# hippylib/hippyflow

Hardware: AMD Instinct MI355X
Metric: randomized-SVD throughput (GDoF*rank/s) (higher is better)
Workload: dtype f64

## Files before the change

### hippyflow_amd/csrc/hfmi_skinny.hip

```cpp
#include "hfmi_internal.h"

typedef double d4 __attribute__((ext_vector_type(4)));
typedef double d2 __attribute__((ext_vector_type(2)));
#define MFMA_F64(a, b, c) __builtin_amdgcn_mfma_f64_16x16x4f64((a), (b), (c), 0, 0, 0)
typedef const __attribute__((address_space(1))) d2* gd2ptr;
typedef const __attribute__((address_space(1))) double* gdptr;

#ifndef SS_NT
#define SS_NT 1
#endif
#if SS_NT
#define SS_LOAD(p) __builtin_nontemporal_load(p)
#else
#define SS_LOAD(p) (*(p))
#endif
#ifndef SS_PROBE
#define SS_PROBE 0
#endif
constexpr int SS_THREADS = 512;

template <int NT, int TPW, int NQ, bool STORE>
__device__ __forceinline__ void ss_stage(const double* __restrict__ L, double* __restrict__ Lnext, const int la,
                                         const int la1, const int (&toa)[TPW], const int (&tob)[TPW],
                                         d4 (&acc)[TPW], const d2 (&r)[NQ], const int dst0) {
  constexpr int CT = NQ * 32;
  constexpr int S = 4 * NT;
  constexpr int W0 = (S >= 8) ? (3 * S) / 4 : 0;
  constexpr int PER = (NQ + (S - W0) - 1) / (S - W0);
  d2 fa[2], fb[2];
  fa[0] = *reinterpret_cast<const d2*>(L + toa[0] + la);
  fb[0] = *reinterpret_cast<const d2*>(L + tob[0] + la);
#pragma unroll
  for (int st = 0; st < S; ++st) {
    if (st + 1 < S) {
      const int it = (st + 1) / NT, ti = (st + 1) % NT;
      const int lx = (it & 1) ? la1 : la;
      fa[(st + 1) & 1] = *reinterpret_cast<const d2*>(L + toa[ti] + lx + it * (8 * CT));
      fb[(st + 1) & 1] = *reinterpret_cast<const d2*>(L + tob[ti] + lx + it * (8 * CT));
    }
    if (STORE && st >= W0) {
#pragma unroll
      for (int j = 0; j < PER; ++j) {
        const int q = (st - W0) * PER + j;
        if (q < NQ) *reinterpret_cast<d2*>(Lnext + dst0 + q * 64) = r[q];
      }
    }
    __builtin_amdgcn_sched_barrier(0);
    const int ti = st % NT;
    acc[ti] = MFMA_F64(fa[st & 1].x, fb[st & 1].x, acc[ti]);
    acc[ti] = MFMA_F64(fa[st & 1].y, fb[st & 1].y, acc[ti]);
    __builtin_amdgcn_sched_barrier(0);
  }
}

__device__ __forceinline__ gdptr ss_colptr(int v, int ctot, int acols, const double* A, int64_t lda, int m,
                                           const double* B, int64_t ldb, int k) {
  const int vv = v < ctot ? v : ctot - 1;
  const double* p;
  if (vv < acols) {
    const int cc = vv < m ? vv : m - 1;
    p = A + (int64_t)cc * lda;
  } else {
    const int cc = (vv - acols) < k ? (vv - acols) : k - 1;
    p = B + (int64_t)cc * ldb;
  }
  return (gdptr)p;
}

template <int NT, int TPW, int NQ, int PF>
__device__ __forceinline__ void ss_main(double* __restrict__ lds, const gdptr* __restrict__ ptab,
                                        const gdptr (&ptr)[NQ], const int nstages, const int col0, const int off,
                                        const int dst0, const int la, const int la1, const int (&toa)[TPW],
                                        const int (&tob)[TPW], d4 (&acc)[TPW]) {
  constexpr int BUF = NQ * 32 * SS_BK;
  d2 reg[PF][NQ];
  auto stage_load = [&](d2(&r)[NQ], int s) {
    if (s > nstages - 1) s = nstages - 1;
#pragma unroll
    for (int q = 0; q < NQ; ++q) {
      if constexpr (PF == 2)
        r[q] = SS_LOAD(reinterpret_cast<gd2ptr>(ptr[q] + (int64_t)s * SS_BK));
      else
        r[q] = SS_LOAD(reinterpret_cast<gd2ptr>(ptab[col0 + 32 * q] + ((int64_t)s * SS_BK + off)));
    }
  };
  if (nstages > 0) {
    stage_load(reg[0], 0);
#pragma unroll
    for (int q = 0; q < NQ; ++q) *reinterpret_cast<d2*>(lds + dst0 + q * 64) = reg[0][q];
    if constexpr (PF == 2) stage_load(reg[0], 1);
    __syncthreads();
  }
  if constexpr (PF == 1) {
    for (int s = 0; s < nstages; ++s) {
      stage_load(reg[0], s + 1);
      __builtin_amdgcn_sched_barrier(0);
      ss_stage<NT, TPW, NQ, true>(lds + (s & 1) * BUF, lds + ((s + 1) & 1) * BUF, la, la1, toa, tob, acc, reg[0], dst0);
      __syncthreads();
    }
  } else {
    auto stage_store = [&](const d2(&r)[NQ]) {
#pragma unroll
      for (int q = 0; q < NQ; ++q) *reinterpret_cast<d2*>(lds + dst0 + q * 64) = r[q];
    };
    for (int s = 0; s < nstages; s += 2) {
      stage_load(reg[1], s + 2);
      __builtin_amdgcn_sched_barrier(0);
      ss_stage<NT, TPW, NQ, false>(lds, lds, la, la1, toa, tob, acc, reg[0], dst0);
      __syncthreads();
      stage_store(reg[0]);
      __syncthreads();
      if (s + 1 < nstages) {
        stage_load(reg[0], s + 3);
        __builtin_amdgcn_sched_barrier(0);
        ss_stage<NT, TPW, NQ, false>(lds, lds, la, la1, toa, tob, acc, reg[1], dst0);
        __syncthreads();
        stage_store(reg[1]);
        __syncthreads();
      }
    }
  }
}

template <int TPW, int NQ, int PF>
__global__ __launch_bounds__(SS_THREADS, (TPW <= 4 ? 4 : 2)) void k_tsgemm_ss(
    const double* __restrict__ A, int64_t lda, int m, int rt, const double* __restrict__ B, int64_t ldb, int k, int ct,
    int same, int64_t Npad, int64_t chunk, double* __restrict__ part) {
  extern __shared__ __attribute__((aligned(16))) char smem[];
  constexpr int CT = NQ * 32;
  constexpr int BUF = CT * SS_BK;
  double* lds = reinterpret_cast<double*>(smem);
  gdptr* ptab = reinterpret_cast<gdptr*>(lds + 2 * BUF);
  const int tid = threadIdx.x, lane = tid & 63;
  const int wave = __builtin_amdgcn_readfirstlane(tid >> 6);
  const int r16 = lane & 15, kk = lane >> 4;
  const int acols = rt * 16;
  const int ctot = same ? acols : acols + ct * 16;
  const int bcol0 = same ? 0 : acols;

  const int64_t t_begin = (int64_t)blockIdx.x * chunk;
  int64_t t_end = t_begin + chunk;
  if (t_end > Npad) t_end = Npad;
  const int nstages = t_end > t_begin ? (int)((t_end - t_begin) / SS_BK) : 0;

  const int col0 = tid >> 4;
  const int cq = tid & 15;
  const int dst0 = (cq * CT + (col0 ^ (cq & 7))) * 2;
  gdptr ptr[NQ];
#pragma unroll
  for (int q = 0; q < NQ; ++q) ptr[q] = nullptr;
  if constexpr (PF == 2) {
#pragma unroll
    for (int q = 0; q < NQ; ++q) ptr[q] = ss_colptr(col0 + 32 * q, ctot, acols, A, lda, m, B, ldb, k) + (t_begin + cq * 2);
  } else {
    for (int v = tid; v < CT; v += SS_THREADS) ptab[v] = ss_colptr(v, ctot, acols, A, lda, m, B, ldb, k) + t_begin;
    __syncthreads();
  }

  const int ntiles = same ? rt * (rt + 1) / 2 : rt * ct;
  const bool last_valid = wave + 8 * (TPW - 1) < ntiles;
  auto tile_rc = [&](int id, int& r, int& c) {
    if (same) {
      r = 0;
      while (id >= rt - r) {
        id -= rt - r;
        ++r;
      }
      c = r + id;
    } else {
      r = id / ct;
      c = id - r * ct;
    }
  };
  int toa[TPW], tob[TPW];
#pragma unroll
  for (int ti = 0; ti < TPW; ++ti) {
    int id = wave + 8 * ti;
    if (id > ntiles - 1) id = ntiles - 1;
    int r, c;
    tile_rc(id, r, c);
    toa[ti] = r * 32;
    tob[ti] = (bcol0 + c * 16) * 2;
  }
  const int la = (kk * CT + (r16 ^ kk)) * 2, la1 = (kk * CT + (r16 ^ (kk + 4))) * 2;
  d4 acc[TPW];
#pragma unroll
  for (int ti = 0; ti < TPW; ++ti) acc[ti] = d4{0.0, 0.0, 0.0, 0.0};

  if (TPW == 1 || last_valid)
    ss_main<TPW, TPW, NQ, PF>(lds, ptab, ptr, nstages, col0, cq * 2, dst0, la, la1, toa, tob, acc);
  else
    ss_main<(TPW > 1 ? TPW - 1 : 1), TPW, NQ, PF>(lds, ptab, ptr, nstages, col0, cq * 2, dst0, la, la1, toa, tob, acc);

  const int kpad = ct * 16;
  double* P = part + (int64_t)blockIdx.x * acols * kpad;
#pragma unroll
  for (int ti = 0; ti < TPW; ++ti) {
    const int id = wave + 8 * ti;
    if (id < ntiles) {
      int r, c;
      tile_rc(id, r, c);
#pragma unroll
      for (int e = 0; e < 4; ++e) P[(int64_t)(r * 16 + kk + 4 * e) * kpad + c * 16 + r16] = acc[ti][e];
      if (same && r != c) {
#pragma unroll
        for (int e = 0; e < 4; ++e) P[(int64_t)(c * 16 + r16) * kpad + r * 16 + kk + 4 * e] = acc[ti][e];
      }
    }
  }
}

template <int RB, int CB, int EN, int NQ>
__device__ __forceinline__ void ssb_stage(const double* __restrict__ L, double* __restrict__ Lnext, const int la, const int la1,
                                          const int (&toa)[RB], const int (&tob)[CB], const int (&etoa)[EN > 0 ? EN : 1],
                                          const int (&etob)[EN > 0 ? EN : 1], d4 (&acc)[RB][CB], d4 (&eacc)[EN > 0 ? EN : 1],
                                          const d2 (&r)[NQ], const int dst0, const int probe_acols = 0) {
  constexpr int CT = NQ * 32;
  constexpr int EA = EN > 0 ? EN : 1;
  (void)probe_acols;
  d2 fa[2][RB], fb[2][CB], ea[2][EA], eb[2][EA];
#pragma unroll
  for (int i = 0; i < RB; ++i) fa[0][i] = *reinterpret_cast<const d2*>(L + toa[i] + la);
#pragma unroll
  for (int j = 0; j < CB; ++j) fb[0][j] = *reinterpret_cast<const d2*>(L + tob[j] + la);
#pragma unroll
  for (int e = 0; e < EN; ++e) {
    ea[0][e] = *reinterpret_cast<const d2*>(L + etoa[e] + la);
    eb[0][e] = *reinterpret_cast<const d2*>(L + etob[e] + la);
  }
#pragma unroll
  for (int it = 0; it < 4; ++it) {
    if (it + 1 < 4) {
      const int lx = (((it + 1) & 1) ? la1 : la) + (it + 1) * (8 * CT);
#pragma unroll
      for (int i = 0; i < RB; ++i) fa[(it + 1) & 1][i] = *reinterpret_cast<const d2*>(L + toa[i] + lx);
#pragma unroll
      for (int j = 0; j < CB; ++j) {
#if SS_PROBE & 2
        fb[(it + 1) & 1][j] = d2{fb[it & 1][j].y, fb[it & 1][j].x};
#else
        fb[(it + 1) & 1][j] = *reinterpret_cast<const d2*>(L + tob[j] + lx);
#endif
      }
#pragma unroll
      for (int e = 0; e < EN; ++e) {
        ea[(it + 1) & 1][e] = *reinterpret_cast<const d2*>(L + etoa[e] + lx);
        eb[(it + 1) & 1][e] = *reinterpret_cast<const d2*>(L + etob[e] + lx);
      }
    }
    if (it >= 2) {
      constexpr int H = (NQ + 1) / 2;
#pragma unroll
      for (int q = (it - 2) * H; q < ((it - 2) * H + H < NQ ? (it - 2) * H + H : NQ); ++q) {
#if SS_PROBE & 1
        if ((int)(threadIdx.x >> 4) + 32 * q >= probe_acols) {
          asm volatile("" ::"v"(r[q].x), "v"(r[q].y));
          continue;
        }
#endif
        *reinterpret_cast<d2*>(Lnext + dst0 + q * 64) = r[q];
      }
    }
    __builtin_amdgcn_sched_barrier(0);
#pragma unroll
    for (int i = 0; i < RB; ++i)
#pragma unroll
      for (int j = 0; j < CB; ++j) acc[i][j] = MFMA_F64(fa[it & 1][i].x, fb[it & 1][j].x, acc[i][j]);
#pragma unroll
    for (int e = 0; e < EN; ++e) eacc[e] = MFMA_F64(ea[it & 1][e].x, eb[it & 1][e].x, eacc[e]);
#pragma unroll
    for (int i = 0; i < RB; ++i)
#pragma unroll
      for (int j = 0; j < CB; ++j) acc[i][j] = MFMA_F64(fa[it & 1][i].y, fb[it & 1][j].y, acc[i][j]);
#pragma unroll
    for (int e = 0; e < EN; ++e) eacc[e] = MFMA_F64(ea[it & 1][e].y, eb[it & 1][e].y, eacc[e]);
    __builtin_amdgcn_sched_barrier(0);
  }
}

template <int RB, int CB, int EN, int NQ>
__device__ __forceinline__ void ssb_stage_pipe(const double* __restrict__ L, double* __restrict__ Lnext, const int la, const int la1,
                                               const int (&toa)[RB], const int (&tob)[CB], const int (&etoa)[EN > 0 ? EN : 1],
                                               const int (&etob)[EN > 0 ? EN : 1], d4 (&acc)[RB][CB], d4 (&eacc)[EN > 0 ? EN : 1],
                                               const d2 (&r)[NQ], const int dst0, d2 (&fa)[2][RB], d2 (&fb)[2][CB],
                                               d2 (&ea)[2][EN > 0 ? EN : 1], d2 (&eb)[2][EN > 0 ? EN : 1], const int probe_acols = 0) {
  constexpr int CT = NQ * 32;
  (void)probe_acols;
#pragma unroll
  for (int it = 0; it < 4; ++it) {
    if (it == 3) __syncthreads();
    {
      const double* src = (it + 1 < 4) ? L : Lnext;
      const int g = (it + 1) & 3;
      const int lx = ((g & 1) ? la1 : la) + g * (8 * CT);
#pragma unroll
      for (int i = 0; i < RB; ++i) fa[(it + 1) & 1][i] = *reinterpret_cast<const d2*>(src + toa[i] + lx);
#pragma unroll
      for (int j = 0; j < CB; ++j) {
#if SS_PROBE & 2
        fb[(it + 1) & 1][j] = d2{fb[it & 1][j].y, fb[it & 1][j].x};
#else
        fb[(it + 1) & 1][j] = *reinterpret_cast<const d2*>(src + tob[j] + lx);
#endif
      }
#pragma unroll
      for (int e = 0; e < EN; ++e) {
        ea[(it + 1) & 1][e] = *reinterpret_cast<const d2*>(src + etoa[e] + lx);
        eb[(it + 1) & 1][e] = *reinterpret_cast<const d2*>(src + etob[e] + lx);
      }
    }
    if (it < 2) {
      constexpr int H = (NQ + 1) / 2;
#pragma unroll
      for (int q = it * H; q < (it * H + H < NQ ? it * H + H : NQ); ++q) {
#if SS_PROBE & 1
        if ((int)(threadIdx.x >> 4) + 32 * q >= probe_acols) {
          asm volatile("" ::"v"(r[q].x), "v"(r[q].y));
          continue;
        }
#endif
        *reinterpret_cast<d2*>(Lnext + dst0 + q * 64) = r[q];
      }
    }
    __builtin_amdgcn_sched_barrier(0);
#pragma unroll
    for (int i = 0; i < RB; ++i)
#pragma unroll
      for (int j = 0; j < CB; ++j) acc[i][j] = MFMA_F64(fa[it & 1][i].x, fb[it & 1][j].x, acc[i][j]);
#pragma unroll
    for (int e = 0; e < EN; ++e) eacc[e] = MFMA_F64(ea[it & 1][e].x, eb[it & 1][e].x, eacc[e]);
#pragma unroll
    for (int i = 0; i < RB; ++i)
#pragma unroll
      for (int j = 0; j < CB; ++j) acc[i][j] = MFMA_F64(fa[it & 1][i].y, fb[it & 1][j].y, acc[i][j]);
#pragma unroll
    for (int e = 0; e < EN; ++e) eacc[e] = MFMA_F64(ea[it & 1][e].y, eb[it & 1][e].y, eacc[e]);
    __builtin_amdgcn_sched_barrier(0);
  }
}

template <int RB, int CB, int EN, int NQ, int PF, int RT, bool PIPE>
__device__ __forceinline__ void ssb_run(double* __restrict__ lds, const gdptr* __restrict__ ptab, const int nstages, const int col0,
                                        const int off, const int dst0, const int la, const int la1, const int row_tile0,
                                        const int col_tile0, const int bcol0, double* __restrict__ P, const int kpad, const int r16,
                                        const int kk, const int ext0, const int ext_col0) {
  constexpr int BUF = NQ * 32 * SS_BK;
  constexpr int EA = EN > 0 ? EN : 1;
  int toa[RB], tob[CB], etoa[EA], etob[EA], er[EA], ec[EA];
#pragma unroll
  for (int i = 0; i < RB; ++i) toa[i] = (row_tile0 + i) * 32;
#pragma unroll
  for (int j = 0; j < CB; ++j) tob[j] = (bcol0 + (col_tile0 + j) * 16) * 2;
#pragma unroll
  for (int e = 0; e < EA; ++e) {
    const int id = ext0 + 8 * e;
    er[e] = id % RT;
    ec[e] = ext_col0 + id / RT;
    etoa[e] = er[e] * 32;
    etob[e] = (bcol0 + ec[e] * 16) * 2;
  }
  d4 acc[RB][CB], eacc[EA];
#pragma unroll
  for (int i = 0; i < RB; ++i)
#pragma unroll
    for (int j = 0; j < CB; ++j) acc[i][j] = d4{0.0, 0.0, 0.0, 0.0};
#pragma unroll
  for (int e = 0; e < EA; ++e) eacc[e] = d4{0.0, 0.0, 0.0, 0.0};
  d2 reg[PF][NQ];
  auto stage_load = [&](d2(&rr)[NQ], int s) {
    if (s > nstages - 1) s = nstages - 1;
#pragma unroll
    for (int q = 0; q < NQ; ++q) rr[q] = SS_LOAD(reinterpret_cast<gd2ptr>(ptab[col0 + 32 * q] + ((int64_t)s * SS_BK + off)));
  };
  if (nstages > 0) {
    stage_load(reg[0], 0);
#pragma unroll
    for (int q = 0; q < NQ; ++q) *reinterpret_cast<d2*>(lds + dst0 + q * 64) = reg[0][q];
    if constexpr (PF == 2) stage_load(reg[0], 1);
    __syncthreads();
  }
  if constexpr (PIPE) {
    d2 fa[2][RB], fb[2][CB], ea[2][EA], eb[2][EA];
#pragma unroll
    for (int i = 0; i < RB; ++i) fa[0][i] = *reinterpret_cast<const d2*>(lds + toa[i] + la);
#pragma unroll
    for (int j = 0; j < CB; ++j) fb[0][j] = *reinterpret_cast<const d2*>(lds + tob[j] + la);
#pragma unroll
    for (int e = 0; e < EN; ++e) {
      ea[0][e] = *reinterpret_cast<const d2*>(lds + etoa[e] + la);
      eb[0][e] = *reinterpret_cast<const d2*>(lds + etob[e] + la);
    }
    if constexpr (PF == 2) {
      for (int s = 0; s < nstages; s += 2) {
        stage_load(reg[1], s + 2);
        __builtin_amdgcn_sched_barrier(0);
        ssb_stage_pipe<RB, CB, EN, NQ>(lds, lds + BUF, la, la1, toa, tob, etoa, etob, acc, eacc, reg[0], dst0, fa, fb, ea, eb, RT * 16);
        if (s + 1 < nstages) {
          stage_load(reg[0], s + 3);
          __builtin_amdgcn_sched_barrier(0);
          ssb_stage_pipe<RB, CB, EN, NQ>(lds + BUF, lds, la, la1, toa, tob, etoa, etob, acc, eacc, reg[1], dst0, fa, fb, ea, eb, RT * 16);
        }
      }
    } else {
      for (int s = 0; s < nstages; ++s) {
        stage_load(reg[0], s + 1);
        __builtin_amdgcn_sched_barrier(0);
        ssb_stage_pipe<RB, CB, EN, NQ>(lds + (s & 1) * BUF, lds + ((s + 1) & 1) * BUF, la, la1, toa, tob, etoa, etob, acc, eacc,
                                       reg[0], dst0, fa, fb, ea, eb, RT * 16);
      }
    }
  } else if constexpr (PF == 2) {
    for (int s = 0; s < nstages; s += 2) {
      stage_load(reg[1], s + 2);
      __builtin_amdgcn_sched_barrier(0);
      ssb_stage<RB, CB, EN, NQ>(lds, lds + BUF, la, la1, toa, tob, etoa, etob, acc, eacc, reg[0], dst0, RT * 16);
      __syncthreads();
      if (s + 1 < nstages) {
        stage_load(reg[0], s + 3);
        __builtin_amdgcn_sched_barrier(0);
        ssb_stage<RB, CB, EN, NQ>(lds + BUF, lds, la, la1, toa, tob, etoa, etob, acc, eacc, reg[1], dst0, RT * 16);
        __syncthreads();
      }
    }
  } else {
    for (int s = 0; s < nstages; ++s) {
      stage_load(reg[0], s + 1);
      __builtin_amdgcn_sched_barrier(0);
      ssb_stage<RB, CB, EN, NQ>(lds + (s & 1) * BUF, lds + ((s + 1) & 1) * BUF, la, la1, toa, tob, etoa, etob, acc, eacc, reg[0], dst0, RT * 16);
      __syncthreads();
    }
  }
#pragma unroll
  for (int i = 0; i < RB; ++i)
#pragma unroll
    for (int j = 0; j < CB; ++j)
#pragma unroll
      for (int e = 0; e < 4; ++e)
        P[(int64_t)((row_tile0 + i) * 16 + kk + 4 * e) * kpad + (col_tile0 + j) * 16 + r16] = acc[i][j][e];
#pragma unroll
  for (int x = 0; x < EN; ++x)
#pragma unroll
    for (int e = 0; e < 4; ++e) P[(int64_t)(er[x] * 16 + kk + 4 * e) * kpad + ec[x] * 16 + r16] = eacc[x][e];
}

template <int RT, int CTL, int NQ, bool PIPE>
__global__ __launch_bounds__(SS_THREADS, 2) void k_tsgemm_ssb(const double* __restrict__ A, int64_t lda, int m,
                                                              const double* __restrict__ B, int64_t ldb, int k, int64_t Npad,
                                                              int64_t chunk, double* __restrict__ part) {
  extern __shared__ __attribute__((aligned(16))) char smem[];
  constexpr int CT = NQ * 32;
  constexpr int BUF = CT * SS_BK;
  constexpr int RB0 = (RT + 1) / 2, RB1 = RT / 2;
  constexpr int CBF = CTL / 4, CM = 4 * CBF, NLEFT = (CTL - CM) * RT;
  static_assert(RB1 >= 1 && CBF >= 1, "blocked variant needs at least 2 x 4 tiles");
  constexpr int ENB_HI = (NLEFT + 7) / 8, ENB_LO = NLEFT / 8 + ((NLEFT % 8) > 3 ? 1 : 0);
  constexpr int ENT_HI = (NLEFT + 3) / 8, ENT_LO = NLEFT > 4 ? (NLEFT - 4) / 8 + (((NLEFT - 4) % 8) > 3 ? 1 : 0) : 0;
  double* lds = reinterpret_cast<double*>(smem);
  gdptr* ptab = reinterpret_cast<gdptr*>(lds + 2 * BUF);
  const int tid = threadIdx.x, lane = tid & 63;
  const int wave = __builtin_amdgcn_readfirstlane(tid >> 6);
  const int r16 = lane & 15, kk = lane >> 4;
  constexpr int acols = RT * 16, ctot = (RT + CTL) * 16;
  const int64_t t_begin = (int64_t)blockIdx.x * chunk;
  int64_t t_end = t_begin + chunk;
  if (t_end > Npad) t_end = Npad;
  const int nstages = t_end > t_begin ? (int)((t_end - t_begin) / SS_BK) : 0;
  const int col0 = tid >> 4, cq = tid & 15;
  const int dst0 = (cq * CT + (col0 ^ (cq & 7))) * 2;
  for (int v = tid; v < CT; v += SS_THREADS) ptab[v] = ss_colptr(v, ctot, acols, A, lda, m, B, ldb, k) + t_begin;
  __syncthreads();
  const int la = (kk * CT + (r16 ^ kk)) * 2, la1 = (kk * CT + (r16 ^ (kk + 4))) * 2;
  const int rg = wave >> 2, cg = wave & 3;
  const int row_tile0 = rg ? RB0 : 0;
  const int col_tile0 = cg * CBF;
  const int ext0 = rg ? cg : cg + 4;
  int en = 0;
  for (int id = ext0; id < NLEFT; id += 8) ++en;
  constexpr int kpad = CTL * 16;
  double* P = part + (int64_t)blockIdx.x * acols * kpad;
  constexpr int PF = (RT * CTL <= 56) ? 2 : 1;
#define SSB_RUN(RBV, ENV) ssb_run<RBV, CBF, ENV, NQ, PF, RT, PIPE>(lds, ptab, nstages, col0, cq * 2, dst0, la, la1, row_tile0, col_tile0, acols, P, kpad, r16, kk, ext0, CM)
  if (rg == 0) {
    if (ENT_HI != ENT_LO && en == ENT_LO) SSB_RUN(RB0, ENT_LO);
    else SSB_RUN(RB0, ENT_HI);
  } else {
    if (ENB_HI != ENB_LO && en == ENB_LO) SSB_RUN(RB1, ENB_LO);
    else SSB_RUN(RB1, ENB_HI);
  }
#undef SSB_RUN
}

typedef void (*ss_kernel_t)(const double*, int64_t, int, int, const double*, int64_t, int, int, int, int64_t, int64_t, double*);
typedef void (*ssb_kernel_t)(const double*, int64_t, int, const double*, int64_t, int, int64_t, int64_t, double*);
static ss_kernel_t ss_kernel(const ss_plan& p) {
#define SS_CASE(T, Q) \
  if (p.tpw == T && p.nq == Q) return k_tsgemm_ss<T, Q, ss_pf(T, Q)>;
  HFMI_SS_CASES(SS_CASE)
#undef SS_CASE
  return nullptr;
}
static ssb_kernel_t ssb_kernel(const ss_plan& p) {
#define SSB_CASE(R, Cc) \
  if (p.rt == R && p.ct == Cc) return p.pipe ? k_tsgemm_ssb<R, Cc, (R + Cc + 1) / 2, true> : k_tsgemm_ssb<R, Cc, (R + Cc + 1) / 2, false>;
  HFMI_SSB_CASES(SSB_CASE)
#undef SSB_CASE
  return nullptr;
}

int launch_tsgemm_ss(hfmi_ctx* ctx, const double* A, int64_t lda, int m, const double* B, int64_t ldb, int k,
                     int64_t N, double scale, double beta, double* C, int64_t rs, int64_t cs, int nsplit_req) {
  const bool same = (A == B && lda == ldb && m == k);
  const ss_plan p = ss_plan_make(m, k, N, same, nsplit_req, tsgemm_knobs_ref(), ctx->num_cus);
  if (lda % 32 != 0 || ldb % 32 != 0 || lda < p.Npad || ldb < p.Npad)
    HFMI_FAIL(HFMI_ERR_INVALID, "tsgemm_ss: leading dimensions must be multiples of 32 and >= round_up(N,32)");
  const ss_kernel_t kern = p.blocked ? nullptr : ss_kernel(p);
  const ssb_kernel_t kern_b = p.blocked ? ssb_kernel(p) : nullptr;
  if (!kern && !kern_b) HFMI_FAIL(HFMI_ERR_INVALID, "tsgemm_ss: no instance for tiles/wave=%d chunks/thread=%d", p.tpw, p.nq);
  void* partv = nullptr;
  HFMI_TRY(ctx_ws(ctx, WS_PART, p.ws_bytes, &partv));
  double* part = (double*)partv;
  const int pidx = prof_start(ctx, 0, m, k, N);
  if (same && pidx >= 0) {
    ctx->prof[pidx].flops = (double)N * k * (k + 1);
    ctx->prof[pidx].bytes = 8.0 * ((double)N * k + (double)k * k);
  }
  HIP_TRY(hipFuncSetAttribute(p.blocked ? (const void*)kern_b : (const void*)kern, hipFuncAttributeMaxDynamicSharedMemorySize, (int)p.shmem));
  if (!p.blocked)
    hipLaunchKernelGGL(kern, dim3(p.nsplit), dim3(SS_THREADS), p.shmem, ctx->stream, A, lda, m, p.swap ? p.ct : p.rt, B, ldb, k,
                       p.swap ? p.rt : p.ct, same ? 1 : 0, p.Npad, p.chunk, part);
  else if (p.swap)
    hipLaunchKernelGGL(kern_b, dim3(p.nsplit), dim3(SS_THREADS), p.shmem, ctx->stream, B, ldb, k, A, lda, m, p.Npad, p.chunk, part);
  else
    hipLaunchKernelGGL(kern_b, dim3(p.nsplit), dim3(SS_THREADS), p.shmem, ctx->stream, A, lda, m, B, ldb, k, p.Npad, p.chunk, part);
  HIP_TRY(hipGetLastError());
  ss_plan_words(p, plan_slot(ctx));
  prof_stop(ctx, pidx);
  return launch_reduce_partials(ctx, part, p.red, scale, beta, C, rs, cs);
}
```

Before: 0.1670.

## Stream skinny-GEMM tiles directly into LDS with a four-deep ring buffer

By default the blocked skinny TSGEMM no longer stages global loads through registers. It issues global_load_lds transfers straight into a four-slot LDS ring of half-depth (16-row) stages, keeping up to three stages in flight and retiring them with explicit vmcnt waits. LDS fragment reads for the next half-stage are interleaved inside the MFMA sequence, and the LDS layout and swizzle are reworked for the new load pattern. The aim is to cut register pressure and VALU copy work and to hide global-memory latency. The cost is finer-grained barriers (twice as many stages) and a dependence on correct manual waitcnt accounting.

Result: no change. 0.1665 (-0.3%).

```diff
diff --git a/hippyflow_amd/csrc/hfmi_skinny.hip b/hippyflow_amd/csrc/hfmi_skinny.hip
--- a/hippyflow_amd/csrc/hfmi_skinny.hip
+++ b/hippyflow_amd/csrc/hfmi_skinny.hip
@@ -210,6 +210,7 @@
   }
 }
 
+#ifdef HFMI_SSB_REGSTAGE
 template <int RB, int CB, int EN, int NQ>
 __device__ __forceinline__ void ssb_stage(const double* __restrict__ L, double* __restrict__ Lnext, const int la, const int la1,
                                           const int (&toa)[RB], const int (&tob)[CB], const int (&etoa)[EN > 0 ? EN : 1],
@@ -442,6 +443,149 @@
 #pragma unroll
     for (int e = 0; e < 4; ++e) P[(int64_t)(er[x] * 16 + kk + 4 * e) * kpad + ec[x] * 16 + r16] = eacc[x][e];
 }
+
+#else
+constexpr int SSB_RK = 16;
+#define SSB_VMCNT(N) asm volatile("s_waitcnt vmcnt(%0)" ::"n"(N) : "memory")
+typedef __attribute__((address_space(3))) void* ldsvptr;
+typedef const __attribute__((address_space(1))) void* gvptr;
+
+template <int LJ>
+__device__ __forceinline__ void ssb_retire(const int keep) {
+  if (keep >= 2) SSB_VMCNT(2 * LJ);
+  else if (keep == 1) SSB_VMCNT(LJ);
+  else SSB_VMCNT(0);
+}
+
+template <int RB, int CB, int EN>
+__device__ __forceinline__ void ssb_frags(const double* __restrict__ L, const int lx, const int (&toa)[RB], const int (&tob)[CB],
+                                          const int (&etoa)[EN > 0 ? EN : 1], const int (&etob)[EN > 0 ? EN : 1], d2 (&fa)[RB],
+                                          d2 (&fb)[CB], d2 (&ea)[EN > 0 ? EN : 1], d2 (&eb)[EN > 0 ? EN : 1]) {
+#pragma unroll
+  for (int i = 0; i < RB; ++i) fa[i] = *reinterpret_cast<const d2*>(L + toa[i] + lx);
+#pragma unroll
+  for (int j = 0; j < CB; ++j) fb[j] = *reinterpret_cast<const d2*>(L + tob[j] + lx);
+#pragma unroll
+  for (int e = 0; e < EN; ++e) {
+    ea[e] = *reinterpret_cast<const d2*>(L + etoa[e] + lx);
+    eb[e] = *reinterpret_cast<const d2*>(L + etob[e] + lx);
+  }
+}
+
+template <int RB, int CB, int EN, class F>
+__device__ __forceinline__ void ssb_mfmas(const d2 (&fa)[RB], const d2 (&fb)[CB], const d2 (&ea)[EN > 0 ? EN : 1],
+                                          const d2 (&eb)[EN > 0 ? EN : 1], d4 (&acc)[RB][CB], d4 (&eacc)[EN > 0 ? EN : 1], F&& reads) {
+  __builtin_amdgcn_sched_barrier(0);
+#pragma unroll
+  for (int i = 0; i < RB; ++i)
+#pragma unroll
+    for (int j = 0; j < CB; ++j) {
+      acc[i][j] = MFMA_F64(fa[i].x, fb[j].x, acc[i][j]);
+      if (i == 0 && j == 0) {
+        __builtin_amdgcn_sched_barrier(0);
+        reads();
+        __builtin_amdgcn_sched_barrier(0);
+      }
+    }
+#pragma unroll
+  for (int e = 0; e < EN; ++e) eacc[e] = MFMA_F64(ea[e].x, eb[e].x, eacc[e]);
+#pragma unroll
+  for (int i = 0; i < RB; ++i)
+#pragma unroll
+    for (int j = 0; j < CB; ++j) acc[i][j] = MFMA_F64(fa[i].y, fb[j].y, acc[i][j]);
+#pragma unroll
+  for (int e = 0; e < EN; ++e) eacc[e] = MFMA_F64(ea[e].y, eb[e].y, eacc[e]);
+  __builtin_amdgcn_sched_barrier(0);
+}
+
+template <int RB, int CB, int EN, int NQ, int LJ, int RT, bool PIPE>
+__device__ __forceinline__ void ssb_run(double* __restrict__ lds, const gdptr* __restrict__ ptab, const int nst, const int wave,
+                                        const int lane, const int row_tile0, const int col_tile0,
+                                        const int bcol0, double* __restrict__ P, const int kpad, const int r16, const int kk,
+                                        const int ext0, const int ext_col0) {
+  constexpr int CT = NQ * 32;
+  constexpr int BUF = CT * SSB_RK;
+  constexpr int EA = EN > 0 ? EN : 1;
+  int toa[RB], tob[CB], etoa[EA], etob[EA], er[EA], ec[EA];
+#pragma unroll
+  for (int i = 0; i < RB; ++i) toa[i] = (row_tile0 + i) * (16 * SSB_RK);
+#pragma unroll
+  for (int j = 0; j < CB; ++j) tob[j] = (bcol0 + (col_tile0 + j) * 16) * SSB_RK;
+#pragma unroll
+  for (int e = 0; e < EA; ++e) {
+    const int id = ext0 + 8 * e;
+    er[e] = id % RT;
+    ec[e] = ext_col0 + id / RT;
+    etoa[e] = er[e] * (16 * SSB_RK);
+    etob[e] = (bcol0 + ec[e] * 16) * SSB_RK;
+  }
+  d4 acc[RB][CB], eacc[EA];
+#pragma unroll
+  for (int i = 0; i < RB; ++i)
+#pragma unroll
+    for (int j = 0; j < CB; ++j) acc[i][j] = d4{0.0, 0.0, 0.0, 0.0};
+#pragma unroll
+  for (int e = 0; e < EA; ++e) eacc[e] = d4{0.0, 0.0, 0.0, 0.0};
+  const int la = (r16 * 8 + (kk ^ (r16 >> 1))) * 2, la1 = (r16 * 8 + ((kk + 4) ^ (r16 >> 1))) * 2;
+  gdptr src[LJ];
+#pragma unroll
+  for (int j = 0; j < LJ; ++j) {
+    const int p = (j * 8 + wave) * 64 + lane;
+    const int v = p >> 3;
+    src[j] = ptab[v] + (((p & 7) ^ ((v >> 1) & 7)) * 2);
+  }
+  auto issue = [&](const int h) {
+    double* dst = lds + (h & 3) * BUF + wave * 128;
+#pragma unroll
+    for (int j = 0; j < LJ; ++j)
+      __builtin_amdgcn_global_load_lds((gvptr)(src[j] + (int64_t)h * SSB_RK), (ldsvptr)(dst + j * 1024), 16, 0, SS_NT ? 2 : 0);
+  };
+  auto keep_after = [&](const int h) {
+    const int k = nst - 1 - h;
+    return k > 2 ? 2 : k;
+  };
+  if (nst > 0) {
+    issue(0);
+    if (nst > 1) issue(1);
+    if (nst > 2) issue(2);
+    ssb_retire<LJ>(keep_after(0));
+    __builtin_amdgcn_s_barrier();
+    d2 fa[2][RB], fb[2][CB], ea[2][EA], eb[2][EA];
+    if constexpr (PIPE) ssb_frags<RB, CB, EN>(lds, la, toa, tob, etoa, etob, fa[0], fb[0], ea[0], eb[0]);
+    for (int h = 0; h < nst; ++h) {
+      const double* L = lds + (h & 3) * BUF;
+      if constexpr (!PIPE) ssb_frags<RB, CB, EN>(L, la, toa, tob, etoa, etob, fa[0], fb[0], ea[0], eb[0]);
+      if (h + 3 < nst) issue(h + 3);
+      ssb_mfmas<RB, CB, EN>(fa[0], fb[0], ea[0], eb[0], acc, eacc,
+                            [&] { ssb_frags<RB, CB, EN>(L, la1, toa, tob, etoa, etob, fa[1], fb[1], ea[1], eb[1]); });
+      if constexpr (PIPE) {
+        ssb_retire<LJ>(keep_after(h + 1));
+        asm volatile("s_waitcnt lgkmcnt(0)" ::: "memory");
+        __builtin_amdgcn_s_barrier();
+        const double* Ln = lds + ((h + 1) & 3) * BUF;
+        ssb_mfmas<RB, CB, EN>(fa[1], fb[1], ea[1], eb[1], acc, eacc,
+                              [&] { ssb_frags<RB, CB, EN>(Ln, la, toa, tob, etoa, etob, fa[0], fb[0], ea[0], eb[0]); });
+      } else {
+        ssb_mfmas<RB, CB, EN>(fa[1], fb[1], ea[1], eb[1], acc, eacc, [] {});
+        ssb_retire<LJ>(keep_after(h + 1));
+        asm volatile("s_waitcnt lgkmcnt(0)" ::: "memory");
+        __builtin_amdgcn_s_barrier();
+      }
+    }
+  }
+#pragma unroll
+  for (int i = 0; i < RB; ++i)
+#pragma unroll
+    for (int j = 0; j < CB; ++j)
+#pragma unroll
+      for (int e = 0; e < 4; ++e)
+        P[(int64_t)((row_tile0 + i) * 16 + kk + 4 * e) * kpad + (col_tile0 + j) * 16 + r16] = acc[i][j][e];
+#pragma unroll
+  for (int x = 0; x < EN; ++x)
+#pragma unroll
+    for (int e = 0; e < 4; ++e) P[(int64_t)(er[x] * 16 + kk + 4 * e) * kpad + ec[x] * 16 + r16] = eacc[x][e];
+}
+#endif
 
 template <int RT, int CTL, int NQ, bool PIPE>
 __global__ __launch_bounds__(SS_THREADS, 2) void k_tsgemm_ssb(const double* __restrict__ A, int64_t lda, int m,
@@ -465,11 +609,8 @@
   int64_t t_end = t_begin + chunk;
   if (t_end > Npad) t_end = Npad;
   const int nstages = t_end > t_begin ? (int)((t_end - t_begin) / SS_BK) : 0;
-  const int col0 = tid >> 4, cq = tid & 15;
-  const int dst0 = (cq * CT + (col0 ^ (cq & 7))) * 2;
   for (int v = tid; v < CT; v += SS_THREADS) ptab[v] = ss_colptr(v, ctot, acols, A, lda, m, B, ldb, k) + t_begin;
   __syncthreads();
-  const int la = (kk * CT + (r16 ^ kk)) * 2, la1 = (kk * CT + (r16 ^ (kk + 4))) * 2;
   const int rg = wave >> 2, cg = wave & 3;
   const int row_tile0 = rg ? RB0 : 0;
   const int col_tile0 = cg * CBF;
@@ -478,14 +619,22 @@
   for (int id = ext0; id < NLEFT; id += 8) ++en;
   constexpr int kpad = CTL * 16;
   double* P = part + (int64_t)blockIdx.x * acols * kpad;
+#ifdef HFMI_SSB_REGSTAGE
   constexpr int PF = (RT * CTL <= 56) ? 2 : 1;
-#define SSB_RUN(RBV, ENV) ssb_run<RBV, CBF, ENV, NQ, PF, RT, PIPE>(lds, ptab, nstages, col0, cq * 2, dst0, la, la1, row_tile0, col_tile0, acols, P, kpad, r16, kk, ext0, CM)
+  const int col0 = tid >> 4, cq = tid & 15;
+  const int dst0 = (cq * CT + (col0 ^ (cq & 7))) * 2;
+  const int la = (kk * CT + (r16 ^ kk)) * 2, la1 = (kk * CT + (r16 ^ (kk + 4))) * 2;
+#define SSB_RUN(RBV, ENV, LJV) ssb_run<RBV, CBF, ENV, NQ, PF, RT, PIPE>(lds, ptab, nstages, col0, cq * 2, dst0, la, la1, row_tile0, col_tile0, acols, P, kpad, r16, kk, ext0, CM)
+#else
+  constexpr int LJ0 = (4 * NQ + 7) / 8, LJ1 = (4 * NQ) / 8;
+#define SSB_RUN(RBV, ENV, LJV) ssb_run<RBV, CBF, ENV, NQ, LJV, RT, PIPE>(lds, ptab, 2 * nstages, wave, lane, row_tile0, col_tile0, acols, P, kpad, r16, kk, ext0, CM)
+#endif
   if (rg == 0) {
-    if (ENT_HI != ENT_LO && en == ENT_LO) SSB_RUN(RB0, ENT_LO);
-    else SSB_RUN(RB0, ENT_HI);
+    if (ENT_HI != ENT_LO && en == ENT_LO) SSB_RUN(RB0, ENT_LO, LJ0);
+    else SSB_RUN(RB0, ENT_HI, LJ0);
   } else {
-    if (ENB_HI != ENB_LO && en == ENB_LO) SSB_RUN(RB1, ENB_LO);
-    else SSB_RUN(RB1, ENB_HI);
+    if (ENB_HI != ENB_LO && en == ENB_LO) SSB_RUN(RB1, ENB_LO, LJ1);
+    else SSB_RUN(RB1, ENB_HI, LJ1);
   }
 #undef SSB_RUN
 }
```
